# cuteboyqq/DPVO

Hardware: AMD Instinct MI355X
Metric: update-iterations/sec (altcorr+fastba) on 96-patch/2048-edge graph, 1→8 GPU (higher is better)
Workload: dtype f32; 1 GPU; cfg2: 96 patches/frame x 2048 edges, p=3, 4-level pyramid [1, 2, 4, 8], fp32 features, BA 2 iters; patches_per_frame=96, edges=2048, frames=12, radius=3, channels=128, feature_ring=36, parallelism=replicas x1

## Files before the change

### dpvo_amd/csrc/ba.hip

```cpp
#include "common.hpp"
#include "ba_device.hpp"

namespace dpvo {

constexpr int kSetupThreads = 1024;
constexpr int kIterThreads = 512;
constexpr int kIterWaves = kIterThreads / 64;
constexpr int kMaxSetupE = 16384;
constexpr int kMaxFree = 20;
constexpr int kPerThread = kMaxSetupE / kSetupThreads;
constexpr int kCtlBytes = 512;
constexpr int kSetupLds = 160 * 1024;
constexpr int kMarks = 2432;
constexpr int kLaunchMarks = 1664;
constexpr int kNoPose = 31;
constexpr int kEC = 16;

struct BaWs {
  int4* srec;
  int32_t* poff;
  int32_t* pu;
  uint32_t* pmask;
  int32_t* meta;
  int64_t* kx;
// ... 256 lines not shown
    work = pij + E;
#pragma unroll
    for (int k = 0; k < kPerThread; k++) {
      const int i = tid + k * T;
      if (i < E) {
        const int e = pe[k];
        const int64_t gi = A.ii[e], gj = A.jj[e];
        const int64_t pi = gi - t0, pj = gj - t0;
        const int ci = (pi >= 0 && pi < N) ? (int)pi : kNoPose;
        const int cj = (pj >= 0 && pj < N) ? (int)pj : kNoPose;
        pij[i] = ci | (cj << 8);
        work[i] = hd[k];
        w.srec[i] = make_int4(e, (int)gi, (int)gj, kv[k]);
      }
    }
    __syncthreads();
    nuniq = block_exclusive_scan(work, E, scr);
#pragma unroll
    for (int k = 0; k < kPerThread; k++) {
      const int i = tid + k * T;
      if (i < E) w.pu[i] = work[i] + hd[k] - 1;
      if (i < E && hd[k]) {
        w.kx[work[i]] = kv[k];
        w.poff[work[i]] = i;
      }
    }
    if (tid == 0) w.poff[nuniq] = E;
  }
  if (tid == 0) {
    w.meta[0] = nuniq;
    w.meta[1] = ctl[0] ? 2 : 0;
    w.meta[3] = A.num_patches;
    w.meta[4] = 0;
  }
  __syncthreads();
  trace(w.tmark, 41);
  for (int u = tid; u < nuniq; u += T) {
    unsigned mask = 0;
    for (int t = w.poff[u]; t < w.poff[u + 1]; t++) {
      const int c = pij[t];
      if ((c & 0xff) != kNoPose) mask |= 1u << (c & 0xff);
      if ((c >> 8) != kNoPose) mask |= 1u << (c >> 8);
    }
    w.pmask[u] = mask;
  }
  trace(w.tmark, 42);
}

#pragma clang fp contract(off)
__device__ __forceinline__ void edge_linearize(const float* poses, const float* patches, int P,
                                               float fx, float fy, float cx, float cy, float tx,
                                               float ty, float wx, float wy, int ix, int jx,
                                               int64_t kx, bool use_depth, float depth, float* o) {
  const float* pk = patches + (size_t)kx * 3 * P * P;
  const int c11 = P + 1;
  const float nx = (pk[c11] - cx) / fx;
  const float ny = (pk[P * P + c11] - cy) / fy;
  const float dz = use_depth ? depth : pk[2 * P * P + c11];
  bad::Lin L;
  bad::lin_edge(poses + 7 * (size_t)ix, poses + 7 * (size_t)jx, nx, ny, dz, tx, ty, wx, wy, fx, fy,
                cx, cy, L);
  o[0] = L.w[0];
  o[1] = L.w[1];
  o[2] = L.r[0];
  o[3] = L.r[1];
  o[4] = L.Jz[0];
  o[5] = L.Jz[1];
#pragma unroll
  for (int a = 0; a < 6; a++) {
    o[6 + a] = L.Ji[0][a];
    o[12 + a] = L.Ji[1][a];
    o[18 + a] = L.Jj[0][a];
    o[24 + a] = L.Jj[1][a];
  }
}

__global__ void reproject_kernel(const float* __restrict__ poses, const float* __restrict__ patches,
                                 const float* __restrict__ intrinsics,
                                 const int64_t* __restrict__ ii, const int64_t* __restrict__ jj,
                                 const int64_t* __restrict__ kk, int E, int P, int num_poses,
                                 int num_patches, float* __restrict__ coords,
                                 int* __restrict__ order, int N2) {
  if (order && blockIdx.x == gridDim.x - 1) {
    __shared__ int bins[kOrderBins + 1];
    const OrderIn q{poses, patches, intrinsics, ii, kk, P, num_poses, num_patches};
    edge_order_block(q, jj, E, N2, order, bins);
    return;
  }
  const int PP = P * P;
  const int t = blockIdx.x * blockDim.x + threadIdx.x;
  if (t >= E * PP) return;
  reproject_pixel(poses, patches, intrinsics, ii, jj, kk, t / PP, t % PP, P, num_poses,
                  num_patches, coords);
}
#pragma clang fp contract(fast)

__device__ __forceinline__ float retract_depth(const BaWs& w, const double* EC, const double* dX,
                                               int t0, int N, double lam, int u, float base) {
  double C = 0.0, Uu = 0.0, ex = 0.0;
  const int p1 = w.poff[u + 1];
#pragma unroll 2
  for (int t = w.poff[u]; t < p1; t++) {
    const double* ec = EC + kEC * (size_t)t;
    const int pi = (int)ec[14], pj = (int)ec[15];
    C += ec[12];
    Uu += ec[13];
    if (pi >= 0 && pi < N)
#pragma unroll
      for (int k = 0; k < 6; k++) ex += ec[k] * dX[6 * pi + k];
    if (pj >= 0 && pj < N)
#pragma unroll
      for (int k = 0; k < 6; k++) ex += ec[6 + k] * dX[6 * pj + k];
  }
  const float dz = (float)((1.0 / (C + lam)) * (Uu - ex));
  float d = base + dz;
  d = (d > 20.0f) ? 1.0f : d;
  return (float)fmax((double)d, 1e-4);
}

__global__ void __launch_bounds__(256) ba_lin_kernel(BaArgs A, BaWs w, int it) {
  const int t = blockIdx.x * blockDim.x + threadIdx.x;
  if (t == 0) w.lam[0] = A.lmbda[0];
  if (t >= A.E) return;
  const float fx = A.intrinsics[0], fy = A.intrinsics[1], cx = A.intrinsics[2],
              cy = A.intrinsics[3];
  const int4 r = w.srec[t];
  const int kmax = w.meta[3] - 1;
  float depth = 0.0f;
  if (it > 0) {
    const int u = w.pu[t], P = A.P;
    const float base = (it == 1)
                           ? A.patches[(size_t)min(r.w, kmax) * 3 * P * P + 2 * P * P]
                           : w.dbuf[(it - 1) & 1][u];
    depth = retract_depth(w, w.EC[(it - 1) & 1], w.dX, A.t0, A.N, (double)A.lmbda[0], u, base);
    if (t == w.poff[u]) w.dbuf[it & 1][u] = depth;
  }
  const float2 tg = reinterpret_cast<const float2*>(A.target)[r.x];
  const float2 wt = reinterpret_cast<const float2*>(A.weight)[r.x];
  const int ix = min(max(r.y, 0), A.num_poses - 1);
  const int jx = min(max(r.z, 0), A.num_poses - 1);
  float o[30];
  edge_linearize(A.poses, A.patches, A.P, fx, fy, cx, cy, tg.x, tg.y, wt.x, wt.y, ix, jx,
                 (int64_t)min(r.w, kmax), it > 0, depth, o);
  float4* Jo = reinterpret_cast<float4*>(w.J + 32 * (size_t)t);
#pragma unroll
  for (int k = 0; k < 7; k++) Jo[k] = make_float4(o[4 * k], o[4 * k + 1], o[4 * k + 2], o[4 * k + 3]);
  reinterpret_cast<float2*>(Jo + 7)[0] = make_float2(o[28], o[29]);
  double ec[kEC];
#pragma unroll
  for (int k = 0; k < 14; k++) ec[k] = 0.0;
#pragma unroll
  for (int row = 0; row < 2; row++) {
    const double wr = o[row];
    const float rr = o[2 + row], Jz = o[4 + row];
    const double wz = wr * Jz;
#pragma unroll
    for (int k = 0; k < 6; k++) {
      ec[k] -= wz * o[6 + 6 * row + k];
      ec[6 + k] += wz * o[18 + 6 * row + k];
    }
    ec[12] += wz * Jz;
    ec[13] += wr * rr * Jz;
  }
  ec[14] = (double)(r.y - A.t0);
  ec[15] = (double)(r.z - A.t0);
  double2* Eo = reinterpret_cast<double2*>(w.EC[it & 1] + kEC * (size_t)t);
#pragma unroll
// ... 947 lines not shown
```

### dpvo_amd/csrc/ba_window.hip

```cpp
#include <unistd.h>

#include <algorithm>
#include <chrono>
#include <cstdio>
#include <random>
#include <cstdlib>
#include <map>
#include <mutex>

#include "ba_solve.hpp"
#include "pyr_insert.hpp"

namespace dpvo {
namespace {
using namespace bad;

constexpr int kWT = 256;
constexpr int kPT = 512;
constexpr int kWMaxN = 16;
constexpr int kWMaxE = 10240;
constexpr int kWMaxG = 256;
constexpr int kWLds = 160 * 1024;
constexpr int kHistMax = 12288;
constexpr int kWSlots = 64;
// ... 325 lines not shown
              k64[lo] = b;
              k64[hi] = a;
            }
          } else {
            const unsigned a = k32[lo], b = k32[hi];
            if ((a > b) == up) {
              k32[lo] = b;
              k32[hi] = a;
            }
          }
        }
        __syncthreads();
      }
    for (int p = tid; p < E; p += T) {
      if (wide) {
        spos[p] = (unsigned short)(k64[p] & 0xffffffffull);
        head[p] = (p == 0 || (k64[p] >> 32) != (k64[p - 1] >> 32)) ? 1 : 0;
      } else {
        spos[p] = (unsigned short)(k32[p] & 0x3fffu);
        head[p] = (p == 0 || (k32[p] >> 14) != (k32[p - 1] >> 14)) ? 1 : 0;
      }
    }
  }
  __syncthreads();
  int* hd = (int*)U;
  for (int p = tid; p < E; p += T) hd[p] = head[p];
  __syncthreads();
  const int nuniq = fscan(hd, E, scr);
  for (int p = tid; p < E; p += T) {
    const int u1 = (p + 1 < E) ? hd[p + 1] : nuniq;
    const bool is_head = u1 != hd[p];
    const int u = u1 - 1;
    const int e = pos_edge[p];
    plan.epos[p] = e;
    if (is_head) {
      plan.poff[u] = p;
      plan.pkk[u] = (int)min(max(kk[e], (int64_t)0), (int64_t)kmaxc);
    }
  }
  if (tid == 0) plan.poff[nuniq] = E;
  unsigned* mask = (unsigned*)(U + sizeof(int) * cap);
  for (int u = tid; u < nuniq; u += T) mask[u] = 0u;
  __syncthreads();
  for (int p = tid; p < E; p += T) {
    const int u = ((p + 1 < E) ? hd[p + 1] : nuniq) - 1;
    const unsigned c = code[pos_edge[p]];
    const unsigned ci = c & 0xff, cj = c >> 8;
    const unsigned m = (ci != kFix ? 1u << ci : 0u) | (cj != kFix ? 1u << cj : 0u);
    if (m) atomicOr(&mask[u], m);
  }
  __syncthreads();
  for (int u = tid; u < nuniq; u += T) plan.pmask[u] = mask[u];
  if (tid == 0) {
    plan.meta[0] = nuniq;
    plan.meta[1] = ctl[2];
    plan.meta[2] = ctl[3];
    plan.meta[3] = 0;
    if (ctl[3] && plan.sink) atomicOr(plan.sink, ctl[3]);
    *plan.status = 0;
  }
}

__host__ __device__ constexpr int plan_shards(int E) {
  return E <= 512 ? 1 : ((E + 511) / 512 < kPlanShardMax ? (E + 511) / 512 : kPlanShardMax);
}
template <int kPer>
__device__ __forceinline__ void plan_sharded_k(const int64_t* __restrict__ ii,
                                             const int64_t* __restrict__ jj,
                                               const int64_t* __restrict__ kk, int E, int num_patches,
                                               int num_poses, int t0, int N, const Plan& plan,
                                               char* lds, int cap, size_t lds_bytes, int s, int S) {
  if (S <= 1) {
    if (s == 0) plan_block(ii, jj, kk, E, num_patches, num_poses, t0, N, plan, lds, cap);
    return;
  }
  if (plan.t0d) t0 = *plan.t0d;
  auto stamp = [&](int q) {
    if (s == 0 && threadIdx.x == 0) {
      reinterpret_cast<int64_t*>(plan.meta + 16)[q] = (int64_t)wall_clock64();
      if (q == 0 || q == 6) reinterpret_cast<int64_t*>(plan.meta + 16)[7 + (q == 6)] = (int64_t)clock64();
    }
  };
  stamp(0);
  const int tid = threadIdx.x, lane = tid & 63, T = kPT;
  int* ctl = (int*)lds;
  int* scr = ctl + 16;
  unsigned short* code = (unsigned short*)(lds + 256);
  unsigned short* spos = code + cap;
  int* hf = reinterpret_cast<int*>(spos + cap);
  int kv[kPer];
  plan_edges_pass<kPer>(ii, jj, kk, E, num_patches, num_poses, t0, N, ctl, code, kv);
  stamp(1);
  const int kmin = ctl[0], R = ctl[1] - kmin + 1;
  const int nlmax = (R + S - 1) / S;
  const bool fits = E > 0 && R <= kHistMax && E < (1 << 14) &&
                    256 + 4 * (size_t)cap + 4 * (size_t)R + 4 * (size_t)nlmax + 4 * kWMaxNB <= lds_bytes;
  if (!fits) {
    if (s == 0) {
      __syncthreads();
      plan_block(ii, jj, kk, E, num_patches, num_poses, t0, N, plan, lds, cap);
    }
    return;
  }
  const int lo = (int)((long long)R * s / S), hi = (int)((long long)R * (s + 1) / S), nl = hi - lo;
  unsigned* pm = reinterpret_cast<unsigned*>(hf + R);
  int* wl = reinterpret_cast<int*>(pm + nl);
  for (int v = tid; v < R; v += T) hf[v] = 0;
  for (int v = tid; v < nl; v += T) pm[v] = 0u;
  for (int v = tid; v < kWMaxNB; v += T) wl[v] = 0;
  if (tid == 0) {
    ctl[4] = 0;
    ctl[5] = 0;
    ctl[6] = 0;
  }
  __syncthreads();
  int nb = 0;
#pragma unroll
  for (int r = 0; r < kPer; r++) {
    const int e = tid + r * T;
    if (e >= E) continue;
    const int v = kv[r] - kmin;
    atomicAdd(&hf[v], 1);
    nb += v < lo ? 1 : 0;
  }
  __syncthreads();
  stamp(2);
  int ub = 0, nu = 0;
  for (int v = tid; v < R; v += T) {
    const int present = hf[v] > 0 ? 1 : 0;
    nu += present;
    ub += v < lo ? present : 0;
  }
  nb = wave_sum_i(nb);
  ub = wave_sum_i(ub);
  nu = wave_sum_i(nu);
  if (lane == 0) {
    atomicAdd(&ctl[4], nb);
    atomicAdd(&ctl[5], ub);
    atomicAdd(&ctl[6], nu);
  }
  int* hist = hf + lo;
  fscan(hist, nl, scr, 14);
  stamp(3);
  const int below = ctl[4], ubelow = ctl[5], nuniq = ctl[6];
#pragma unroll
  for (int r = 0; r < kPer; r++) {
    const int e = tid + r * T;
    const int v = kv[r] - kmin - lo;
    if (e >= E || v < 0 || v >= nl) continue;
    const int old = atomicAdd(&hist[v], 1 << 14);
    spos[old >> 14] = (unsigned short)e;
    const unsigned c = code[e], ci = c & 0xff, cj = c >> 8;
    const unsigned m = (ci != kFix ? 1u << ci : 0u) | (cj != kFix ? 1u << cj : 0u);
    if (m) atomicOr(&pm[old & 0x3fff], m);
  }
  __syncthreads();
  stamp(4);
  plan_block_work(nl, [&](int v, int& c, unsigned& m) {
    const int hv = hist[v];
    c = (hv >> 14) - (v == 0 ? 0 : (hist[v - 1] >> 14));
    m = pm[hv & 0x3fff];
  }, wl);
  stamp(5);
#pragma unroll
  for (int r = 0; r < kPer; r++) {
    const int e = tid + r * T;
    const int v = kv[r] - kmin - lo;
    if (e >= E || v < 0 || v >= nl) continue;
    const int hv = hist[v];
    const int b = hv >> 14, a = (v == 0) ? 0 : (hist[v - 1] >> 14);
    const int rank = bucket_rank(spos, a, b, e);
    plan.epos[below + a + rank] = e;
    if (rank == 0) {
      const int u = ubelow + (hv & 0x3fff);
      plan.poff[u] = below + a;
      plan.pkk[u] = kv[r];
      plan.pmask[u] = pm[hv & 0x3fff];
    }
  }
  __syncthreads();
  plan_store_work(plan, wl, s, N);
  if (tid == 0 && s == S - 1) plan.poff[nuniq] = E;
  if (tid == 0 && s == 0) {
    plan.meta[0] = nuniq;
    plan.meta[1] = ctl[2];
    plan.meta[2] = ctl[3];
    plan.meta[3] = S;
    if (ctl[3] && plan.sink) atomicOr(plan.sink, ctl[3]);
    *plan.status = 0;
  }
  stamp(6);
}

__device__ __forceinline__ void plan_sharded(const int64_t* __restrict__ ii,
                                             const int64_t* __restrict__ jj,
                                             const int64_t* __restrict__ kk, int E, int num_patches,
                                             int num_poses, int t0, int N, const Plan& plan,
                                             char* lds, int cap, size_t lds_bytes, int s, int S) {
  if (E <= 4 * kPT)
    plan_sharded_k<4>(ii, jj, kk, E, num_patches, num_poses, t0, N, plan, lds, cap, lds_bytes, s, S);
  else
    plan_sharded_k<kPlanPer>(ii, jj, kk, E, num_patches, num_poses, t0, N, plan, lds, cap,
                             lds_bytes, s, S);
}

__global__ void __launch_bounds__(kPT) ba_plan_kernel(const int64_t* __restrict__ ii,
                                                      const int64_t* __restrict__ jj,
                                                      const int64_t* __restrict__ kk, int E,
                                                      int num_patches, int num_poses, int t0, int N,
                                                      Plan plan) {
  extern __shared__ __attribute__((aligned(16))) char lds[];
  plan_sharded(ii, jj, kk, E, num_patches, num_poses, t0, N, plan, lds, kWMaxE, kWLds, blockIdx.x,
               gridDim.x);
}

struct RArgs {
  const float* poses;
  const float* patches;
  const float* intrinsics;
  const int64_t* ii;
  const int64_t* jj;
  const int64_t* kk;
  int E, P, num_poses, num_patches, N2, t0, N;
  float* coords;
  int* order;
  int nps;
  int64_t* marks;
};

__global__ void __launch_bounds__(kPT) reproject_plan_kernel(RArgs R, Plan plan) {
  extern __shared__ __attribute__((aligned(16))) char lds[];
  if ((int)blockIdx.x < R.nps) {
    plan_sharded(R.ii, R.jj, R.kk, R.E, R.num_patches, R.num_poses, R.t0, R.N, plan, lds, kWMaxE,
                 kWLds, blockIdx.x, R.nps);
    return;
  }
  if ((int)blockIdx.x == R.nps) {
    const OrderIn q{R.poses, R.patches, R.intrinsics, R.ii, R.kk, R.P, R.num_poses, R.num_patches};
    edge_order_block(q, R.jj, R.E, R.N2, R.order, reinterpret_cast<int*>(lds));
    return;
  }
  const int PP = R.P * R.P;
  const int t = (blockIdx.x - R.nps - 1) * kPT + threadIdx.x;
  if (t >= R.E * PP) return;
  reproject_pixel(R.poses, R.patches, R.intrinsics, R.ii, R.jj, R.kk, t / PP, t % PP, R.P,
                  R.num_poses, R.num_patches, R.coords);
}

struct InsArgs {
  const void* src;
  InsLevels lv;
  int L, C, H, W, gx, gy, ntile;
};

template <typename T>
__device__ __forceinline__ void reproject_plan_insert_body(const RArgs& R, const Plan& plan,
                                                           const InsArgs& I, int nrep, char* lds) {
  const int b = blockIdx.x, b0 = R.nps + 1;
  if (b <= R.nps) __builtin_amdgcn_s_setprio(3);
  if (b < R.nps) {
    plan_sharded(R.ii, R.jj, R.kk, R.E, R.num_patches, R.num_poses, R.t0, R.N, plan, lds,
                 plan_cap(R.E), plan_lds_bytes(plan_cap(R.E)), b, R.nps);
    return;
  }
  if (b == R.nps) {
    const OrderIn q{R.poses, R.patches, R.intrinsics, R.ii, R.kk, R.P, R.num_poses, R.num_patches};
    edge_order_block(q, R.jj, R.E, R.N2, R.order, reinterpret_cast<int*>(lds));
    return;
  }
  if (b < b0 + nrep) {
    const int PP = R.P * R.P;
    const int t = (b - b0) * kPT + threadIdx.x;
    if (t >= R.E * PP) return;
    reproject_pixel(R.poses, R.patches, R.intrinsics, R.ii, R.jj, R.kk, t / PP, t % PP, R.P,
                    R.num_poses, R.num_patches, R.coords);
    return;
  }
  static_assert(kPT == 512, "two 256-thread insertion tiles per workgroup");
  const int half = threadIdx.x >> 8, t = 2 * (b - b0 - nrep) + half;
  const bool act = t < I.ntile;
  const int tt = act ? t : 0;
  float* tile = reinterpret_cast<float*>(lds) + half * kInsTC * kInsCS;
  ins_tile<T>(static_cast<const T*>(I.src), I.lv, I.L, I.C, I.H, I.W, tt % I.gx,
              (tt / I.gx) % I.gy, tt / (I.gx * I.gy), threadIdx.x & 255, act, tile);
}

template <typename T>
__global__ void __launch_bounds__(kPT) reproject_plan_insert_kernel(RArgs R, Plan plan, InsArgs I,
                                                                    int nrep) {
  extern __shared__ __attribute__((aligned(16))) char lds[];
  const bool mk = R.marks && blockIdx.x < 256;
  if (mk && threadIdx.x == 0) R.marks[2 * blockIdx.x] = (int64_t)wall_clock64();
  reproject_plan_insert_body<T>(R, plan, I, nrep, lds);
  if (mk) {
    __syncthreads();
    if (threadIdx.x == 0) R.marks[2 * blockIdx.x + 1] = (int64_t)wall_clock64();
  }
}

struct WL {
  int* ctl;
  float* pose;
  double* dX;
  unsigned short* tri;
  int* roff;
  float2* nxy;
  float* dep;
  float* dbase;
  double2* qu;
  int* pkx;
  unsigned short* ec;
  unsigned short* rp;
  int* eid;
  float4* tw;
  float* ej;
  char* region;
  __device__ __forceinline__ void ld_ej(const float* ejg, int E, int q, int par, float4& e0,
                                        float4& e1, float4& e2) const {
    if (ej) {
      const float4* e4 = reinterpret_cast<const float4*>(ej + 12 * (size_t)q);
      e0 = e4[0];
      e1 = e4[1];
      e2 = e4[2];
    } else {
      const __amdgpu_buffer_rsrc_t rs = __builtin_amdgcn_make_buffer_rsrc(
          const_cast<float*>(ejg), 0, (int)(sizeof(float) * 24 * (size_t)E), kBufDword3);
      const int o = (int)(sizeof(float) * 12 * ((size_t)par * E + eid[q]));
      e0 = __builtin_bit_cast(float4, __builtin_amdgcn_raw_buffer_load_b128(rs, o, 0, kSc1));
      e1 = __builtin_bit_cast(float4, __builtin_amdgcn_raw_buffer_load_b128(rs, o + 16, 0, kSc1));
      e2 = __builtin_bit_cast(float4, __builtin_amdgcn_raw_buffer_load_b128(rs, o + 32, 0, kSc1));
    }
  }
};

enum { cNrel = 0, cNrp = 1, cFmin = 2, cFail = 3, cTimeout = 4, cCap = 5, cFailAny = 6, cLMulti = 7,
       cScan = 16 };

__device__ __forceinline__ double edges_etdx(const WL& L, const WArgs& A, int q0, int q1, int par,
                                             int N) {
  constexpr int kEb = 4;
  double ex = 0.0;
  for (int qb = q0; qb < q1; qb += kEb) {
    float4 e[kEb][3];
    unsigned cc[kEb];
#pragma unroll
    for (int u = 0; u < kEb; u++) {
      const int q = min(qb + u, q1 - 1);
      cc[u] = L.ec[q];
      L.ld_ej(A.ejg, A.E, q, par, e[u][0], e[u][1], e[u][2]);
    }
#pragma unroll
    for (int u = 0; u < kEb; u++) {
      const bool live = qb + u < q1;
      const unsigned si = cc[u] & 0xff, sj = cc[u] >> 8;
      const unsigned nm = (unsigned)max(N - 1, 0);
      const double* dj = L.dX + 6 * min(sj, nm);
      const double* di = L.dX + 6 * min(si, nm);
      const float4 e0 = e[u][0], e1 = e[u][1], e2 = e[u][2];
      const double tj = (double)e0.x * dj[0] + (double)e0.y * dj[1] + (double)e0.z * dj[2] +
                        (double)e0.w * dj[3] + (double)e1.x * dj[4] + (double)e1.y * dj[5];
      const double ti = (double)e1.z * di[0] + (double)e1.w * di[1] + (double)e2.x * di[2] +
                        (double)e2.y * di[3] + (double)e2.z * di[4] + (double)e2.w * di[5];
      ex += (live && sj < (unsigned)N) ? tj : 0.0;
      ex += (live && si < (unsigned)N) ? ti : 0.0;
    }
  }
  return ex;
}
__device__ __forceinline__ double patch_etdx(const WL& L, const WArgs& A, int ri, int par, int N) {
  return edges_etdx(L, A, L.roff[ri], L.roff[ri + 1], par, N);
}
// ... 1013 lines not shown
  g_sink[dev] = sink;
}

void ba_window_plan_offsets(int E, int64_t* out) {
  out[0] = 0;
  out[1] = out[0] + (int64_t)al256w(sizeof(int) * (size_t)E);
  out[2] = out[1] + (int64_t)al256w(sizeof(int) * (size_t)(E + 1));
  out[3] = out[2] + (int64_t)al256w(sizeof(unsigned) * (size_t)E);
  out[4] = out[3] + (int64_t)al256w(sizeof(int) * (size_t)E);
}

static Plan plan_view(char* scratch, int E, int* status) {
  Plan p;
  char* s = scratch;
  p.epos = (int*)s;
  s += al256w(sizeof(int) * (size_t)E);
  p.poff = (int*)s;
  s += al256w(sizeof(int) * (size_t)(E + 1));
  p.pmask = (unsigned*)s;
  s += al256w(sizeof(unsigned) * (size_t)E);
  p.pkk = (int*)s;
  s += al256w(sizeof(int) * (size_t)E);
  p.meta = (int*)s;
  p.status = status;
  p.sink = sink_for_device();
  p.t0d = nullptr;
  return p;
}

static void set_attrs() {
  static bool attr = false;
  if (!attr) {
    (void)hipFuncSetAttribute((const void*)ba_window_kernel,
                              hipFuncAttributeMaxDynamicSharedMemorySize, kWLds);
    (void)hipFuncSetAttribute((const void*)ba_plan_kernel,
                              hipFuncAttributeMaxDynamicSharedMemorySize, kWLds);
    (void)hipFuncSetAttribute((const void*)reproject_plan_kernel,
                              hipFuncAttributeMaxDynamicSharedMemorySize, kWLds);
    (void)hipFuncSetAttribute((const void*)reproject_plan_insert_kernel<float>,
                              hipFuncAttributeMaxDynamicSharedMemorySize, kWLds);
    (void)hipFuncSetAttribute((const void*)reproject_plan_insert_kernel<__half>,
                              hipFuncAttributeMaxDynamicSharedMemorySize, kWLds);
    attr = true;
  }
}

int ba_window_plan(const int64_t* ii, const int64_t* jj, const int64_t* kk, int E, int num_patches,
                   int num_poses, int t0, int t1, char* scratch, int* status, void* stream,
                   const int* t0d) {
  set_attrs();
  Plan plan = plan_view(scratch, E, status);
  plan.t0d = t0d;
  hipLaunchKernelGGL(ba_plan_kernel, dim3(plan_shards(E)), dim3(kPT), kWLds, as_stream(stream), ii, jj, kk, E,
                     num_patches, num_poses, t0, t1 - t0, plan);
  return launch_status();
}

int ba_window_reproject_plan(const float* poses, const float* patches, const float* intrinsics,
                             const int64_t* ii, const int64_t* jj, const int64_t* kk, int E, int P,
                             int num_poses, int num_patches, int N2, float* coords, int* order,
                             int t0, int t1, char* scratch, int* status, void* stream,
                             const int* t0d) {
  set_attrs();
  Plan plan = plan_view(scratch, E, status);
  plan.t0d = t0d;
  RArgs r;
  r.marks = nullptr;
  r.poses = poses;
  r.patches = patches;
  r.intrinsics = intrinsics;
  r.ii = ii;
  r.jj = jj;
  r.kk = kk;
  r.E = E;
  r.P = P;
  r.num_poses = num_poses;
  r.num_patches = num_patches;
  r.N2 = N2;
  r.t0 = t0;
  r.N = t1 - t0;
  r.coords = coords;
  r.order = order;
  r.nps = plan_shards(E);
  const int total = E * P * P;
  hipLaunchKernelGGL(reproject_plan_kernel, dim3(r.nps + 1 + (total + kPT - 1) / kPT), dim3(kPT), kWLds,
                     as_stream(stream), r, plan);
  return launch_status();
}

int ba_window_reproject_plan_insert(const float* poses, const float* patches,
                                    const float* intrinsics, const int64_t* ii, const int64_t* jj,
                                    const int64_t* kk, int E, int P, int num_poses,
                                    int num_patches, int N2, float* coords, int* order, int t0,
                                    int t1, char* scratch, int* status, const void* src,
                                    void* const* dst, const int* scale, int L, int C, int H, int W,
                                    int half, int64_t* marks, void* stream) {
  set_attrs();
  Plan plan = plan_view(scratch, E, status);
  plan.t0d = nullptr;
  RArgs r;
  r.marks = marks;
  r.poses = poses;
  r.patches = patches;
  r.intrinsics = intrinsics;
  r.ii = ii;
  r.jj = jj;
  r.kk = kk;
  r.E = E;
  r.P = P;
  r.num_poses = num_poses;
  r.num_patches = num_patches;
  r.N2 = N2;
  r.t0 = t0;
  r.N = t1 - t0;
  r.coords = coords;
  r.order = order;
  r.nps = plan_shards(E);
  InsArgs I = {};
  I.src = src;
  I.L = L;
  I.C = C;
  I.H = H;
  I.W = W;
  I.lv.mem = 1;
  for (int l = 0; l < L; l++) {
    I.lv.dst[l] = dst[l];
    I.lv.s[l] = scale[l];
  }
  I.gx = (W + kInsTX - 1) / kInsTX;
  I.gy = (H + kInsTY - 1) / kInsTY;
  I.ntile = I.gx * I.gy * ((C + kInsTC - 1) / kInsTC);
  const int nrep = (E * P * P + kPT - 1) / kPT;
  const dim3 grid(r.nps + 1 + nrep + (I.ntile + 1) / 2);
  size_t lds = plan_lds_bytes(plan_cap(E));
  lds = std::max(lds, sizeof(float) * 2 * kInsTC * kInsCS);
  lds = std::max(lds, sizeof(int) * (size_t)(kOrderBins + 2));
  if (half)
    hipLaunchKernelGGL(reproject_plan_insert_kernel<__half>, grid, dim3(kPT), lds,
                       as_stream(stream), r, plan, I, nrep);
  else
    hipLaunchKernelGGL(reproject_plan_insert_kernel<float>, grid, dim3(kPT), lds,
                       as_stream(stream), r, plan, I, nrep);
  return launch_status();
}

int ba_window_run(float* poses, float* patches, const float* intrinsics, const float* target,
                  const float* weight, const float* lmbda, const int64_t* ii, const int64_t* jj,
                  const int64_t* kk, int E, int P, int num_poses, int num_patches, int t0, int t1,
                  int iterations, char* scratch, int* status, int64_t* marks, double* dxo,
                  void* stream, const int* t0d = nullptr);

int ba_window_launch(float* poses, float* patches, const float* intrinsics, const float* target,
                     const float* weight, const float* lmbda, const int64_t* ii, const int64_t* jj,
                     const int64_t* kk, int E, int P, int num_poses, int num_patches, int t0, int t1,
                     int iterations, char* scratch, int* status, int64_t* marks, double* dxo,
                     void* stream) {
  const int rc = ba_window_plan(ii, jj, kk, E, num_patches, num_poses, t0, t1, scratch, status,
                                stream, nullptr);
  if (rc) return rc;
  return ba_window_run(poses, patches, intrinsics, target, weight, lmbda, ii, jj, kk, E, P,
                       num_poses, num_patches, t0, t1, iterations, scratch, status, marks, dxo,
                       stream);
}

int ba_window_run(float* poses, float* patches, const float* intrinsics, const float* target,
                  const float* weight, const float* lmbda, const int64_t* ii, const int64_t* jj,
                  const int64_t* kk, int E, int P, int num_poses, int num_patches, int t0, int t1,
                  int iterations, char* scratch, int* status, int64_t* marks, double* dxo,
                  void* stream, const int* t0d) {
  set_attrs();
  if (iterations > 63) return DPVO_ERR_UNSUPPORTED;
  const int N = t1 - t0;
  const WGrid w = window_grid(E, N);
  hipStream_t st = as_stream(stream);
  WArgs a;
  a.flags = wflag_slot(st);
  if (!a.flags) return DPVO_ERR_LAUNCH;
  a.plan = plan_view(scratch, E, status);
  char* s = scratch + al256w(sizeof(int) * (size_t)E) + al256w(sizeof(int) * (size_t)(E + 1)) +
            al256w(sizeof(unsigned) * (size_t)E) + al256w(sizeof(int) * (size_t)E) +
            al256w(kMetaBytes);
  a.part = (double*)s;
  s += al256w(sizeof(double) * 2 * kPartPad * (size_t)w.G);
  a.gran = (v4u*)s;
  s += al256w((size_t)16 * gran_count(w));
  a.ejg = (float*)s;
  a.poses = poses;
  a.patches = patches;
  a.intrinsics = intrinsics;
  a.target = target;
  a.weight = weight;
  a.lmbda = lmbda;
  a.ii = ii;
  a.jj = jj;
  a.kk = kk;
  a.E = E;
  a.P = P;
  a.num_poses = num_poses;
  a.num_patches = num_patches;
  a.t0 = t0;
  a.t0d = t0d;
  a.N = N;
  a.iters = iterations;
  a.NB = w.NB;
  a.Sd = w.Sd;
  a.So = w.So;
  a.G = w.G;
  a.status = status;
  a.sink = a.plan.sink;
  a.marks = marks;
  a.dxo = dxo;
  a.salt = granule_salt();
  hipLaunchKernelGGL(ba_window_kernel, dim3(w.G), dim3(kWT), kWLds, st, a);
  return launch_status();
}

}
```

### dpvo_amd/csrc/common.hpp

```cpp
#pragma once

#include <hip/hip_fp16.h>
#include <hip/hip_runtime.h>
#include <stdint.h>

#include "dpvo_hot.h"

#define DPVO_EXPORT extern "C" __attribute__((visibility("default")))

namespace dpvo {

constexpr int kWave = 64;
constexpr int kMaxDevices = 64;

inline hipStream_t as_stream(void* s) { return reinterpret_cast<hipStream_t>(s); }

inline int launch_status() {
  hipError_t e = hipGetLastError();
  return e == hipSuccess ? DPVO_OK : DPVO_ERR_LAUNCH;
}

template <typename T>
struct Acc { using type = float; };
template <>
struct Acc<double> { using type = double; };

__device__ __forceinline__ float to_acc(float v) { return v; }
__device__ __forceinline__ float to_acc(__half v) { return __half2float(v); }
__device__ __forceinline__ double to_acc(double v) { return v; }

template <typename T>
__device__ __forceinline__ T from_acc(float v);
template <>
__device__ __forceinline__ float from_acc<float>(float v) { return v; }
template <>
__device__ __forceinline__ __half from_acc<__half>(float v) { return __float2half(v); }
template <>
__device__ __forceinline__ double from_acc<double>(float v) { return (double)v; }
__device__ __forceinline__ double from_acc_d(double v) { return v; }

__device__ __forceinline__ int ifloor_safe(float v) {
  float f = floorf(v);
  f = fminf(fmaxf(f, -1.0e8f), 1.0e8f);
  return (int)f;
}

__device__ __forceinline__ int wave_uniform(int v) { return __builtin_amdgcn_readfirstlane(v); }

__device__ __forceinline__ void wave_lds_sync() {
  __builtin_amdgcn_fence(__ATOMIC_ACQ_REL, "wavefront", "local");
  __builtin_amdgcn_wave_barrier();
}

template <typename Op>
__device__ __forceinline__ int wave_scan_dpp(int x, int id, Op op) {
  x = op(x, __builtin_amdgcn_update_dpp(id, x, 0x111, 0xf, 0xf, false));
  x = op(x, __builtin_amdgcn_update_dpp(id, x, 0x112, 0xf, 0xf, false));
  x = op(x, __builtin_amdgcn_update_dpp(id, x, 0x114, 0xf, 0xf, false));
  x = op(x, __builtin_amdgcn_update_dpp(id, x, 0x118, 0xf, 0xf, false));
  x = op(x, __builtin_amdgcn_update_dpp(id, x, 0x142, 0xa, 0xf, false));
  x = op(x, __builtin_amdgcn_update_dpp(id, x, 0x143, 0xc, 0xf, false));
  return x;
}
__device__ __forceinline__ int wave_incl_sum(int x) {
  return wave_scan_dpp(x, 0, [](int a, int b) { return a + b; });
}
__device__ __forceinline__ int wave_sum_i(int x) {
  return __builtin_amdgcn_readlane(wave_incl_sum(x), 63);
}
__device__ __forceinline__ int wave_min_i(int x) {
  return __builtin_amdgcn_readlane(
      wave_scan_dpp(x, 0x7fffffff, [](int a, int b) { return a < b ? a : b; }), 63);
}
__device__ __forceinline__ int wave_max_i(int x) {
  return __builtin_amdgcn_readlane(
      wave_scan_dpp(x, (int)0x80000000, [](int a, int b) { return a > b ? a : b; }), 63);
}

template <typename T>
__device__ __forceinline__ T wave_sum(T v) {
#pragma unroll
  for (int o = 32; o > 0; o >>= 1) v += __shfl_xor(v, o, kWave);
  return v;
}

#pragma clang fp contract(off)
__device__ __forceinline__ void actSO3(const float* q, const float* X, float* Y) {
  float uv[3];
  uv[0] = 2.0f * (q[1] * X[2] - q[2] * X[1]);
  uv[1] = 2.0f * (q[2] * X[0] - q[0] * X[2]);
  uv[2] = 2.0f * (q[0] * X[1] - q[1] * X[0]);
  Y[0] = X[0] + q[3] * uv[0] + (q[1] * uv[2] - q[2] * uv[1]);
  Y[1] = X[1] + q[3] * uv[1] + (q[2] * uv[0] - q[0] * uv[2]);
  Y[2] = X[2] + q[3] * uv[2] + (q[0] * uv[1] - q[1] * uv[0]);
}

__device__ __forceinline__ void actSE3(const float* t, const float* q, const float* X, float* Y) {
  actSO3(q, X, Y);
  Y[3] = X[3];
  Y[0] += X[3] * t[0];
  Y[1] += X[3] * t[1];
  Y[2] += X[3] * t[2];
}

__device__ __forceinline__ void adjSE3(const float* t, const float* q, const float* X, float* Y) {
  float qinv[4] = {-q[0], -q[1], -q[2], q[3]};
  actSO3(qinv, &X[0], &Y[0]);
  actSO3(qinv, &X[3], &Y[3]);
  float u[3], v[3];
  u[0] = t[2] * X[1] - t[1] * X[2];
  u[1] = t[0] * X[2] - t[2] * X[0];
  u[2] = t[1] * X[0] - t[0] * X[1];
  actSO3(qinv, u, v);
  Y[3] += v[0];
  Y[4] += v[1];
  Y[5] += v[2];
}

__device__ __forceinline__ void relSE3(const float* ti, const float* qi, const float* tj,
                                       const float* qj, float* tij, float* qij) {
  qij[0] = -qj[3] * qi[0] + qj[0] * qi[3] - qj[1] * qi[2] + qj[2] * qi[1];
  qij[1] = -qj[3] * qi[1] + qj[1] * qi[3] - qj[2] * qi[0] + qj[0] * qi[2];
  qij[2] = -qj[3] * qi[2] + qj[2] * qi[3] - qj[0] * qi[1] + qj[1] * qi[0];
  qij[3] = qj[3] * qi[3] + qj[0] * qi[0] + qj[1] * qi[1] + qj[2] * qi[2];
  actSO3(qij, ti, tij);
  tij[0] = tj[0] - tij[0];
  tij[1] = tj[1] - tij[1];
  tij[2] = tj[2] - tij[2];
}

__device__ __forceinline__ void expSO3(const float* phi, float* q) {
  float theta_sq = phi[0] * phi[0] + phi[1] * phi[1] + phi[2] * phi[2];
  float theta_p4 = theta_sq * theta_sq;
  float theta = sqrtf(theta_sq);
// ... 44 lines not shown
}

__device__ __forceinline__ void retrSE3(const float* xi, const float* t, const float* q, float* t1,
                                        float* q1) {
  float dt[3] = {0, 0, 0};
  float dq[4] = {0, 0, 0, 1};
  expSE3(xi, dt, dq);
  q1[0] = dq[3] * q[0] + dq[0] * q[3] + dq[1] * q[2] - dq[2] * q[1];
  q1[1] = dq[3] * q[1] + dq[1] * q[3] + dq[2] * q[0] - dq[0] * q[2];
  q1[2] = dq[3] * q[2] + dq[2] * q[3] + dq[0] * q[1] - dq[1] * q[0];
  q1[3] = dq[3] * q[3] - dq[0] * q[0] - dq[1] * q[1] - dq[2] * q[2];
  actSO3(dq, t, t1);
  t1[0] += dt[0];
  t1[1] += dt[1];
  t1[2] += dt[2];
}

__device__ __forceinline__ void reproject_uv(const float* __restrict__ poses,
                                             const float* __restrict__ patches,
                                             const float* __restrict__ intrinsics,
                                             const int64_t* __restrict__ ii,
                                             const int64_t* __restrict__ jj,
                                             const int64_t* __restrict__ kk, int n, int pix, int P,
                                             int num_poses, int num_patches, float& u, float& v) {
  const int PP = P * P;
  const float fx = intrinsics[0], fy = intrinsics[1], cx = intrinsics[2], cy = intrinsics[3];
  const int ix = (int)min(max(ii[n], (int64_t)0), (int64_t)num_poses - 1);
  const int jx = (int)min(max(jj[n], (int64_t)0), (int64_t)num_poses - 1);
  const int64_t kx = min(max(kk[n], (int64_t)0), (int64_t)num_patches - 1);
  const float* pi = poses + 7 * (size_t)ix;
  const float* pj = poses + 7 * (size_t)jx;
  float ti[3] = {pi[0], pi[1], pi[2]}, qi[4] = {pi[3], pi[4], pi[5], pi[6]};
  float tj[3] = {pj[0], pj[1], pj[2]}, qj[4] = {pj[3], pj[4], pj[5], pj[6]};
  float tij[3], qij[4];
  relSE3(ti, qi, tj, qj, tij, qij);
  const float* pk = patches + (size_t)kx * 3 * PP;
  float Xi[4], Xj[4];
  Xi[0] = (pk[pix] - cx) / fx;
  Xi[1] = (pk[PP + pix] - cy) / fy;
  Xi[2] = 1.0f;
  Xi[3] = pk[2 * PP + pix];
  actSE3(tij, qij, Xi, Xj);
  u = fx * (Xj[0] / Xj[2]) + cx;
  v = fy * (Xj[1] / Xj[2]) + cy;
}

__device__ __forceinline__ void reproject_pixel(const float* __restrict__ poses,
                                                const float* __restrict__ patches,
                                                const float* __restrict__ intrinsics,
                                                const int64_t* __restrict__ ii,
                                                const int64_t* __restrict__ jj,
                                                const int64_t* __restrict__ kk, int n, int pix,
                                                int P, int num_poses, int num_patches,
                                                float* __restrict__ coords) {
  const int PP = P * P;
  float u, v;
  reproject_uv(poses, patches, intrinsics, ii, jj, kk, n, pix, P, num_poses, num_patches, u, v);
  coords[((size_t)n * 2 + 0) * PP + pix] = u;
  coords[((size_t)n * 2 + 1) * PP + pix] = v;
}

#pragma clang fp contract(fast)

struct OrderIn {
  const float* poses;
  const float* patches;
  const float* intrinsics;
  const int64_t* ii;
  const int64_t* kk;
  int P, num_poses, num_patches;
};
constexpr int kOrderBins = 1024;
constexpr int kOrderBands = 16;
__device__ __forceinline__ int edge_order_key(const OrderIn& q, const int64_t* __restrict__ jj,
                                              int e, int nf) {
  const int64_t f = jj[e];
  float u, v;
  const int c = (q.P / 2) * q.P + q.P / 2;
  reproject_uv(q.poses, q.patches, q.intrinsics, q.ii, jj, q.kk, e, c, q.P, q.num_poses,
               q.num_patches, u, v);
  const int band = v >= 0.0f ? (int)fminf(v * (1.0f / 16.0f), (float)(kOrderBands - 1)) : 0;
  return ((f >= 0 && f < nf) ? (int)f : nf - 1) * kOrderBands + band;
}
__device__ inline void edge_order_block(const OrderIn& q, const int64_t* __restrict__ jj, int E,
                                        int N2, int* __restrict__ order, int* bins) {
  const int tid = threadIdx.x, T = blockDim.x;
  const int nf = min(max(N2, 1), kOrderBins / kOrderBands), nb = nf * kOrderBands;
  if (E <= 0) return;
  auto keys4 = [&](int e0, int (&k)[4]) __attribute__((always_inline)) {
#pragma unroll
    for (int r = 0; r < 4; r++) k[r] = edge_order_key(q, jj, min(e0 + r * T, E - 1), nf);
  };
  int k0[4];
  keys4(tid, k0);
  for (int b = tid; b <= nb; b += T) bins[b] = 0;
  __syncthreads();
  for (int e0 = tid; e0 < E; e0 += 4 * T) {
    int k[4];
    if (e0 == tid) {
#pragma unroll
      for (int r = 0; r < 4; r++) k[r] = k0[r];
    } else {
      keys4(e0, k);
    }
#pragma unroll
    for (int r = 0; r < 4; r++)
      if (e0 + r * T < E) atomicAdd(&bins[k[r]], 1);
  }
  __syncthreads();
  if (tid < 64) {
    int carry = 0;
    for (int b0 = 0; b0 < nb; b0 += 64) {
      const int b = b0 + tid;
      const int c = (b < nb) ? bins[b] : 0;
      int x = c;
#pragma unroll
      for (int o = 1; o < 64; o <<= 1) {
        const int y = __shfl_up(x, o, 64);
        if (tid >= o) x += y;
      }
      if (b < nb) bins[b] = carry + x - c;
      carry += __shfl(x, 63, 64);
    }
  }
  __syncthreads();
  for (int e0 = tid; e0 < E; e0 += 4 * T) {
    int k[4];
    if (e0 == tid) {
#pragma unroll
      for (int r = 0; r < 4; r++) k[r] = k0[r];
    } else {
      keys4(e0, k);
    }
#pragma unroll
    for (int r = 0; r < 4; r++)
      if (e0 + r * T < E) order[atomicAdd(&bins[k[r]], 1)] = e0 + r * T;
  }
}

}
```

Baseline: 8768 update-iterations/s.

## Restructure plan sharding, edge ordering scan, and block placement in reproject-plan kernels

The sharded planner now does a single fused load pass over ii/jj/kk with a hashed full-range histogram, replacing the separate edge pass, per-shard histogram and fscan with a block-wide packed count/unique prefix scan, and iterates output by sorted position. Edge ordering replaces the single-wave serial scan with a block-wide scan and reuses keys computed once. Plan/order blocks are spread across block indices so they land on different compute units, launch bounds request two workgroups per CU, and raw barriers replace __syncthreads. These target the latency of the serial planning chain that gates each update iteration, at the cost of more complex index mapping, a hash mask that falls back when the key range exceeds the table, and added register pressure.

```diff
diff --git a/dpvo_amd/csrc/ba.hip b/dpvo_amd/csrc/ba.hip
--- a/dpvo_amd/csrc/ba.hip
+++ b/dpvo_amd/csrc/ba.hip
@@ -362,7 +362,7 @@
                                  int num_patches, float* __restrict__ coords,
                                  int* __restrict__ order, int N2) {
   if (order && blockIdx.x == gridDim.x - 1) {
-    __shared__ int bins[kOrderBins + 1];
+    __shared__ int bins[kOrderLds];
     const OrderIn q{poses, patches, intrinsics, ii, kk, P, num_poses, num_patches};
     edge_order_block(q, jj, E, N2, order, bins);
     return;
diff --git a/dpvo_amd/csrc/ba_window.hip b/dpvo_amd/csrc/ba_window.hip
--- a/dpvo_amd/csrc/ba_window.hip
+++ b/dpvo_amd/csrc/ba_window.hip
@@ -431,20 +431,87 @@
     }
   };
   stamp(0);
-  const int tid = threadIdx.x, lane = tid & 63, T = kPT;
+  const int tid = threadIdx.x, lane = tid & 63, wid = tid >> 6, T = kPT;
   int* ctl = (int*)lds;
   int* scr = ctl + 16;
-  unsigned short* code = (unsigned short*)(lds + 256);
-  unsigned short* spos = code + cap;
-  int* hf = reinterpret_cast<int*>(spos + cap);
+  unsigned short* spos = (unsigned short*)(lds + 256);
+  unsigned short* sv = spos + cap;
+  int* wl = reinterpret_cast<int*>(sv + cap);
+  int* hf = wl + kWMaxNB;
+  const int avail = (int)((lds_bytes - 256 - 4 * (size_t)cap) / 4) - kWMaxNB;
+  int Z = 16384;
+  while (Z > 64 && Z + ((Z / S + 8) & ~3) > avail) Z >>= 1;
+  const int zm = Z - 1, pmN = (Z / S + 8) & ~3;
+  unsigned* pm = reinterpret_cast<unsigned*>(hf + Z);
+  const int kmaxc = num_patches - 1;
+  constexpr int kRound = kPer % 5 == 0 ? 5 : kPer;
+  static_assert(kPer % kRound == 0, "load rounds");
   int kv[kPer];
-  plan_edges_pass<kPer>(ii, jj, kk, E, num_patches, num_poses, t0, N, ctl, code, kv);
-  stamp(1);
-  const int kmin = ctl[0], R = ctl[1] - kmin + 1;
-  const int nlmax = (R + S - 1) / S;
-  const bool fits = E > 0 && R <= kHistMax && E < (1 << 14) &&
-                    256 + 4 * (size_t)cap + 4 * (size_t)R + 4 * (size_t)nlmax + 4 * kWMaxNB <= lds_bytes;
-  if (!fits) {
+  unsigned mk[kPer];
+  int kmin = 0x7fffffff, kmax = -1, fmin = 0x7fffffff, bad = 0;
+#pragma unroll
+  for (int r = 0; r < kPer; r++) {
+    kv[r] = 0;
+    mk[r] = 0u;
+  }
+#pragma unroll
+  for (int r0 = 0; r0 < kPer; r0 += kRound) {
+    if (r0 > 0 && r0 * T >= E) break;
+    int64_t vk[kRound], vi[kRound], vj[kRound];
+#pragma unroll
+    for (int r = 0; r < kRound; r++) {
+      const int e = min(tid + (r0 + r) * T, E - 1);
+      vk[r] = kk[e];
+      vi[r] = ii[e];
+      vj[r] = jj[e];
+    }
+    if (r0 == 0) {
+      int4* z = reinterpret_cast<int4*>(wl);
+      for (int q = tid; q < (kWMaxNB + Z + pmN) / 4; q += T) z[q] = make_int4(0, 0, 0, 0);
+      if (tid == 0) {
+        ctl[0] = 0x7fffffff;
+        ctl[1] = -1;
+        ctl[2] = 0x7fffffff;
+        ctl[3] = 0;
+      }
+      lds_barrier();
+      stamp(1);
+    }
+#pragma unroll
+    for (int r = 0; r < kRound; r++) {
+      const int e = tid + (r0 + r) * T;
+      if (e >= E) continue;
+      int64_t v = vk[r];
+      if (v < 0 || v > kmaxc) {
+        bad = 1;
+        v = v < 0 ? 0 : kmaxc;
+      }
+      kmin = min(kmin, (int)v);
+      kmax = max(kmax, (int)v);
+      kv[r0 + r] = (int)v;
+      atomicAdd(&hf[(int)v & zm], 1);
+      const int64_t gi = vi[r], gj = vj[r];
+      const bool fi = gi >= t0 && gi < t0 + N, fj = gj >= t0 && gj < t0 + N;
+      if (!fi) fmin = min(fmin, (int)min(max(gi, (int64_t)0), (int64_t)num_poses - 1));
+      if (!fj) fmin = min(fmin, (int)min(max(gj, (int64_t)0), (int64_t)num_poses - 1));
+      mk[r0 + r] = (fi ? 1u << (int)(gi - t0) : 0u) | (fj ? 1u << (int)(gj - t0) : 0u);
+    }
+  }
+  kmin = wave_min_i(kmin);
+  kmax = wave_max_i(kmax);
+  fmin = wave_min_i(fmin);
+  bad = wave_max_i(bad);
+  if (lane == 0) {
+    atomicMin(&ctl[0], kmin);
+    atomicMax(&ctl[1], kmax);
+    atomicMin(&ctl[2], fmin);
+    if (bad) atomicOr(&ctl[3], kStClamp);
+  }
+  lds_barrier();
+  stamp(2);
+  kmin = ctl[0];
+  const int R = ctl[1] - kmin + 1;
+  if (__builtin_expect(R > Z || E >= (1 << 14), 0)) {
     if (s == 0) {
       __syncthreads();
       plan_block(ii, jj, kk, E, num_patches, num_poses, t0, N, plan, lds, cap);
@@ -452,82 +519,74 @@
     return;
   }
   const int lo = (int)((long long)R * s / S), hi = (int)((long long)R * (s + 1) / S), nl = hi - lo;
-  unsigned* pm = reinterpret_cast<unsigned*>(hf + R);
-  int* wl = reinterpret_cast<int*>(pm + nl);
-  for (int v = tid; v < R; v += T) hf[v] = 0;
-  for (int v = tid; v < nl; v += T) pm[v] = 0u;
-  for (int v = tid; v < kWMaxNB; v += T) wl[v] = 0;
-  if (tid == 0) {
-    ctl[4] = 0;
-    ctl[5] = 0;
-    ctl[6] = 0;
-  }
-  __syncthreads();
-  int nb = 0;
-#pragma unroll
-  for (int r = 0; r < kPer; r++) {
-    const int e = tid + r * T;
-    if (e >= E) continue;
-    const int v = kv[r] - kmin;
-    atomicAdd(&hf[v], 1);
-    nb += v < lo ? 1 : 0;
-  }
-  __syncthreads();
-  stamp(2);
-  int ub = 0, nu = 0;
-  for (int v = tid; v < R; v += T) {
-    const int present = hf[v] > 0 ? 1 : 0;
-    nu += present;
-    ub += v < lo ? present : 0;
-  }
-  nb = wave_sum_i(nb);
-  ub = wave_sum_i(ub);
-  nu = wave_sum_i(nu);
-  if (lane == 0) {
-    atomicAdd(&ctl[4], nb);
-    atomicAdd(&ctl[5], ub);
-    atomicAdd(&ctl[6], nu);
-  }
-  int* hist = hf + lo;
-  fscan(hist, nl, scr, 14);
+  const int per = (R + T - 1) / T, v0 = tid * per, v1 = min(v0 + per, R);
+  int sum = 0;
+  for (int k0 = v0; k0 < v1; k0 += 4) {
+    int c[4];
+#pragma unroll
+    for (int j = 0; j < 4; j++) c[j] = hf[(kmin + min(k0 + j, v1 - 1)) & zm];
+#pragma unroll
+    for (int j = 0; j < 4; j++) sum += k0 + j < v1 ? (c[j] << 14) | (c[j] > 0 ? 1 : 0) : 0;
+  }
+  const int incl = wave_incl_sum(sum);
+  if (lane == 63) scr[wid] = incl;
+  lds_barrier();
+  int total = 0, run = incl - sum;
+#pragma unroll
+  for (int w = 0; w < kPT / 64; w++) {
+    const int x = scr[w];
+    total += x;
+    run += w < wid ? x : 0;
+  }
+  for (int k0 = v0; k0 < v1; k0 += 4) {
+    int c[4];
+#pragma unroll
+    for (int j = 0; j < 4; j++) c[j] = hf[(kmin + min(k0 + j, v1 - 1)) & zm];
+#pragma unroll
+    for (int j = 0; j < 4; j++) {
+      const int v = k0 + j;
+      if (v >= v1) continue;
+      if (v >= lo && v < hi) hf[(kmin + v) & zm] = run;
+      if (v == lo) ctl[4] = run >> 14;
+      if (v == hi) ctl[5] = run >> 14;
+      run += (c[j] << 14) | (c[j] > 0 ? 1 : 0);
+    }
+  }
+  lds_barrier();
   stamp(3);
-  const int below = ctl[4], ubelow = ctl[5], nuniq = ctl[6];
+  const int nuniq = total & 0x3fff;
+  const int below = ctl[4], top = hi < R ? ctl[5] : total >> 14;
 #pragma unroll
   for (int r = 0; r < kPer; r++) {
     const int e = tid + r * T;
     const int v = kv[r] - kmin - lo;
     if (e >= E || v < 0 || v >= nl) continue;
-    const int old = atomicAdd(&hist[v], 1 << 14);
-    spos[old >> 14] = (unsigned short)e;
-    const unsigned c = code[e], ci = c & 0xff, cj = c >> 8;
-    const unsigned m = (ci != kFix ? 1u << ci : 0u) | (cj != kFix ? 1u << cj : 0u);
-    if (m) atomicOr(&pm[old & 0x3fff], m);
-  }
-  __syncthreads();
+    const int p = atomicAdd(&hf[kv[r] & zm], 1 << 14) >> 14;
+    spos[p] = (unsigned short)e;
+    sv[p] = (unsigned short)v;
+    if (mk[r]) atomicOr(&pm[v], mk[r]);
+  }
+  lds_barrier();
   stamp(4);
   plan_block_work(nl, [&](int v, int& c, unsigned& m) {
-    const int hv = hist[v];
-    c = (hv >> 14) - (v == 0 ? 0 : (hist[v - 1] >> 14));
-    m = pm[hv & 0x3fff];
+    c = (hf[(kmin + lo + v) & zm] >> 14) - (v == 0 ? below : (hf[(kmin + lo + v - 1) & zm] >> 14));
+    m = pm[v];
   }, wl);
   stamp(5);
-#pragma unroll
-  for (int r = 0; r < kPer; r++) {
-    const int e = tid + r * T;
-    const int v = kv[r] - kmin - lo;
-    if (e >= E || v < 0 || v >= nl) continue;
-    const int hv = hist[v];
-    const int b = hv >> 14, a = (v == 0) ? 0 : (hist[v - 1] >> 14);
+  for (int p = below + tid; p < top; p += T) {
+    const int e = spos[p], v = sv[p];
+    const int hv = hf[(kmin + lo + v) & zm];
+    const int b = hv >> 14, a = v == 0 ? below : (hf[(kmin + lo + v - 1) & zm] >> 14);
     const int rank = bucket_rank(spos, a, b, e);
-    plan.epos[below + a + rank] = e;
+    plan.epos[a + rank] = e;
     if (rank == 0) {
-      const int u = ubelow + (hv & 0x3fff);
-      plan.poff[u] = below + a;
-      plan.pkk[u] = kv[r];
-      plan.pmask[u] = pm[hv & 0x3fff];
-    }
-  }
-  __syncthreads();
+      const int u = hv & 0x3fff;
+      plan.poff[u] = a;
+      plan.pkk[u] = kmin + lo + v;
+      plan.pmask[u] = pm[v];
+    }
+  }
+  lds_barrier();
   plan_store_work(plan, wl, s, N);
   if (tid == 0 && s == S - 1) plan.poff[nuniq] = E;
   if (tid == 0 && s == 0) {
@@ -541,16 +600,23 @@
   stamp(6);
 }
 
+__device__ __forceinline__ void plan_sharded_long(const int64_t* __restrict__ ii,
+                                               const int64_t* __restrict__ jj,
+                                               const int64_t* __restrict__ kk, int E, int num_patches,
+                                               int num_poses, int t0, int N, const Plan& plan,
+                                               char* lds, int cap, size_t lds_bytes, int s, int S) {
+  plan_sharded_k<kPlanPer>(ii, jj, kk, E, num_patches, num_poses, t0, N, plan, lds, cap, lds_bytes,
+                           s, S);
+}
 __device__ __forceinline__ void plan_sharded(const int64_t* __restrict__ ii,
                                              const int64_t* __restrict__ jj,
                                              const int64_t* __restrict__ kk, int E, int num_patches,
                                              int num_poses, int t0, int N, const Plan& plan,
                                              char* lds, int cap, size_t lds_bytes, int s, int S) {
-  if (E <= 4 * kPT)
+  if (__builtin_expect(E <= 4 * kPT, 1))
     plan_sharded_k<4>(ii, jj, kk, E, num_patches, num_poses, t0, N, plan, lds, cap, lds_bytes, s, S);
   else
-    plan_sharded_k<kPlanPer>(ii, jj, kk, E, num_patches, num_poses, t0, N, plan, lds, cap,
-                             lds_bytes, s, S);
+    plan_sharded_long(ii, jj, kk, E, num_patches, num_poses, t0, N, plan, lds, cap, lds_bytes, s, S);
 }
 
 __global__ void __launch_bounds__(kPT) ba_plan_kernel(const int64_t* __restrict__ ii,
@@ -574,23 +640,36 @@
   float* coords;
   int* order;
   int nps;
+  int spread;
   int64_t* marks;
 };
 
+__device__ __forceinline__ int launch_chain(const RArgs& R, int b) {
+  if (!R.spread) return b <= R.nps ? b : -1;
+  const int c = 2 * (b >> 3) + (b & 7);
+  return ((b & 7) < 2 && c <= R.nps) ? c : -1;
+}
+__device__ __forceinline__ int launch_rest(const RArgs& R, int b) {
+  if (!R.spread) return b - R.nps - 1;
+  return b - min(R.nps + 1, 2 * (b >> 3) + min(b & 7, 2));
+}
+inline int launch_spread(int nps, int grid) { return grid >= 8 * (nps / 2) + 2 ? 1 : 0; }
+
 __global__ void __launch_bounds__(kPT) reproject_plan_kernel(RArgs R, Plan plan) {
   extern __shared__ __attribute__((aligned(16))) char lds[];
-  if ((int)blockIdx.x < R.nps) {
+  const int chain = launch_chain(R, blockIdx.x);
+  if (chain >= 0 && chain < R.nps) {
     plan_sharded(R.ii, R.jj, R.kk, R.E, R.num_patches, R.num_poses, R.t0, R.N, plan, lds, kWMaxE,
-                 kWLds, blockIdx.x, R.nps);
+                 kWLds, chain, R.nps);
     return;
   }
-  if ((int)blockIdx.x == R.nps) {
+  if (chain == R.nps) {
     const OrderIn q{R.poses, R.patches, R.intrinsics, R.ii, R.kk, R.P, R.num_poses, R.num_patches};
     edge_order_block(q, R.jj, R.E, R.N2, R.order, reinterpret_cast<int*>(lds));
     return;
   }
   const int PP = R.P * R.P;
-  const int t = (blockIdx.x - R.nps - 1) * kPT + threadIdx.x;
+  const int t = launch_rest(R, blockIdx.x) * kPT + threadIdx.x;
   if (t >= R.E * PP) return;
   reproject_pixel(R.poses, R.patches, R.intrinsics, R.ii, R.jj, R.kk, t / PP, t % PP, R.P,
                   R.num_poses, R.num_patches, R.coords);
@@ -605,28 +684,29 @@
 template <typename T>
 __device__ __forceinline__ void reproject_plan_insert_body(const RArgs& R, const Plan& plan,
                                                            const InsArgs& I, int nrep, char* lds) {
-  const int b = blockIdx.x, b0 = R.nps + 1;
-  if (b <= R.nps) __builtin_amdgcn_s_setprio(3);
-  if (b < R.nps) {
+  const int chain = launch_chain(R, blockIdx.x);
+  if (chain >= 0) __builtin_amdgcn_s_setprio(3);
+  if (chain >= 0 && chain < R.nps) {
     plan_sharded(R.ii, R.jj, R.kk, R.E, R.num_patches, R.num_poses, R.t0, R.N, plan, lds,
-                 plan_cap(R.E), plan_lds_bytes(plan_cap(R.E)), b, R.nps);
+                 plan_cap(R.E), plan_lds_bytes(plan_cap(R.E)), chain, R.nps);
     return;
   }
-  if (b == R.nps) {
+  if (chain == R.nps) {
     const OrderIn q{R.poses, R.patches, R.intrinsics, R.ii, R.kk, R.P, R.num_poses, R.num_patches};
     edge_order_block(q, R.jj, R.E, R.N2, R.order, reinterpret_cast<int*>(lds));
     return;
   }
-  if (b < b0 + nrep) {
+  const int b = launch_rest(R, blockIdx.x);
+  if (b < nrep) {
     const int PP = R.P * R.P;
-    const int t = (b - b0) * kPT + threadIdx.x;
+    const int t = b * kPT + threadIdx.x;
     if (t >= R.E * PP) return;
     reproject_pixel(R.poses, R.patches, R.intrinsics, R.ii, R.jj, R.kk, t / PP, t % PP, R.P,
                     R.num_poses, R.num_patches, R.coords);
     return;
   }
   static_assert(kPT == 512, "two 256-thread insertion tiles per workgroup");
-  const int half = threadIdx.x >> 8, t = 2 * (b - b0 - nrep) + half;
+  const int half = threadIdx.x >> 8, t = 2 * (b - nrep) + half;
   const bool act = t < I.ntile;
   const int tt = act ? t : 0;
   float* tile = reinterpret_cast<float*>(lds) + half * kInsTC * kInsCS;
@@ -635,7 +715,7 @@
 }
 
 template <typename T>
-__global__ void __launch_bounds__(kPT) reproject_plan_insert_kernel(RArgs R, Plan plan, InsArgs I,
+__global__ void __launch_bounds__(kPT, 2) reproject_plan_insert_kernel(RArgs R, Plan plan, InsArgs I,
                                                                     int nrep) {
   extern __shared__ __attribute__((aligned(16))) char lds[];
   const bool mk = R.marks && blockIdx.x < 256;
@@ -1815,9 +1895,10 @@
   r.coords = coords;
   r.order = order;
   r.nps = plan_shards(E);
-  const int total = E * P * P;
-  hipLaunchKernelGGL(reproject_plan_kernel, dim3(r.nps + 1 + (total + kPT - 1) / kPT), dim3(kPT), kWLds,
-                     as_stream(stream), r, plan);
+  const int total = E * P * P, grid = r.nps + 1 + (total + kPT - 1) / kPT;
+  r.spread = launch_spread(r.nps, grid);
+  hipLaunchKernelGGL(reproject_plan_kernel, dim3(grid), dim3(kPT), kWLds, as_stream(stream), r,
+                     plan);
   return launch_status();
 }
 
@@ -1865,9 +1946,10 @@
   I.ntile = I.gx * I.gy * ((C + kInsTC - 1) / kInsTC);
   const int nrep = (E * P * P + kPT - 1) / kPT;
   const dim3 grid(r.nps + 1 + nrep + (I.ntile + 1) / 2);
+  r.spread = launch_spread(r.nps, (int)grid.x);
   size_t lds = plan_lds_bytes(plan_cap(E));
   lds = std::max(lds, sizeof(float) * 2 * kInsTC * kInsCS);
-  lds = std::max(lds, sizeof(int) * (size_t)(kOrderBins + 2));
+  lds = std::max(lds, sizeof(int) * (size_t)kOrderLds);
   if (half)
     hipLaunchKernelGGL(reproject_plan_insert_kernel<__half>, grid, dim3(kPT), lds,
                        as_stream(stream), r, plan, I, nrep);
diff --git a/dpvo_amd/csrc/common.hpp b/dpvo_amd/csrc/common.hpp
--- a/dpvo_amd/csrc/common.hpp
+++ b/dpvo_amd/csrc/common.hpp
@@ -50,6 +50,12 @@
 __device__ __forceinline__ void wave_lds_sync() {
   __builtin_amdgcn_fence(__ATOMIC_ACQ_REL, "wavefront", "local");
   __builtin_amdgcn_wave_barrier();
+}
+
+__device__ __forceinline__ void lds_barrier() {
+  __builtin_amdgcn_fence(__ATOMIC_RELEASE, "workgroup", "local");
+  __builtin_amdgcn_s_barrier();
+  __builtin_amdgcn_fence(__ATOMIC_ACQUIRE, "workgroup", "local");
 }
 
 template <typename Op>
@@ -260,60 +266,56 @@
   const int band = v >= 0.0f ? (int)fminf(v * (1.0f / 16.0f), (float)(kOrderBands - 1)) : 0;
   return ((f >= 0 && f < nf) ? (int)f : nf - 1) * kOrderBands + band;
 }
+__device__ __forceinline__ void edge_order_rest(const OrderIn& q, const int64_t* __restrict__ jj, int E,
+                                             int nf, int* __restrict__ order, int* bins) {
+  const int tid = threadIdx.x, T = blockDim.x;
+  for (int e0 = tid + 4 * T; e0 < E; e0 += 4 * T) {
+    int k[4];
+#pragma unroll
+    for (int r = 0; r < 4; r++) k[r] = edge_order_key(q, jj, min(e0 + r * T, E - 1), nf);
+#pragma unroll
+    for (int r = 0; r < 4; r++) {
+      if (e0 + r * T >= E) continue;
+      const int p = atomicAdd(&bins[k[r]], 1);
+      if (order) order[p] = e0 + r * T;
+    }
+  }
+}
+constexpr int kOrderLds = kOrderBins + 1 + 16;
 __device__ inline void edge_order_block(const OrderIn& q, const int64_t* __restrict__ jj, int E,
                                         int N2, int* __restrict__ order, int* bins) {
-  const int tid = threadIdx.x, T = blockDim.x;
+  const int tid = threadIdx.x, T = blockDim.x, lane = tid & 63, wid = tid >> 6;
   const int nf = min(max(N2, 1), kOrderBins / kOrderBands), nb = nf * kOrderBands;
+  int* scr = bins + kOrderBins + 1;
   if (E <= 0) return;
-  auto keys4 = [&](int e0, int (&k)[4]) __attribute__((always_inline)) {
-#pragma unroll
-    for (int r = 0; r < 4; r++) k[r] = edge_order_key(q, jj, min(e0 + r * T, E - 1), nf);
-  };
   int k0[4];
-  keys4(tid, k0);
+#pragma unroll
+  for (int r = 0; r < 4; r++) k0[r] = edge_order_key(q, jj, min(tid + r * T, E - 1), nf);
   for (int b = tid; b <= nb; b += T) bins[b] = 0;
-  __syncthreads();
-  for (int e0 = tid; e0 < E; e0 += 4 * T) {
-    int k[4];
-    if (e0 == tid) {
-#pragma unroll
-      for (int r = 0; r < 4; r++) k[r] = k0[r];
-    } else {
-      keys4(e0, k);
-    }
-#pragma unroll
-    for (int r = 0; r < 4; r++)
-      if (e0 + r * T < E) atomicAdd(&bins[k[r]], 1);
+  lds_barrier();
+#pragma unroll
+  for (int r = 0; r < 4; r++)
+    if (tid + r * T < E) atomicAdd(&bins[k0[r]], 1);
+  if (__builtin_expect(E > 4 * T, 0)) edge_order_rest(q, jj, E, nf, nullptr, bins);
+  lds_barrier();
+  const int per = (nb + T - 1) / T, b0 = min(tid * per, nb), b1 = min(b0 + per, nb);
+  int sum = 0;
+  for (int b = b0; b < b1; b++) sum += bins[b];
+  const int incl = wave_incl_sum(sum);
+  if (lane == 63) scr[wid] = incl;
+  lds_barrier();
+  int run = incl - sum;
+  for (int w = 0; w < wid; w++) run += scr[w];
+  for (int b = b0; b < b1; b++) {
+    const int c = bins[b];
+    bins[b] = run;
+    run += c;
   }
-  __syncthreads();
-  if (tid < 64) {
-    int carry = 0;
-    for (int b0 = 0; b0 < nb; b0 += 64) {
-      const int b = b0 + tid;
-      const int c = (b < nb) ? bins[b] : 0;
-      int x = c;
-#pragma unroll
-      for (int o = 1; o < 64; o <<= 1) {
-        const int y = __shfl_up(x, o, 64);
-        if (tid >= o) x += y;
-      }
-      if (b < nb) bins[b] = carry + x - c;
-      carry += __shfl(x, 63, 64);
-    }
-  }
-  __syncthreads();
-  for (int e0 = tid; e0 < E; e0 += 4 * T) {
-    int k[4];
-    if (e0 == tid) {
-#pragma unroll
-      for (int r = 0; r < 4; r++) k[r] = k0[r];
-    } else {
-      keys4(e0, k);
-    }
-#pragma unroll
-    for (int r = 0; r < 4; r++)
-      if (e0 + r * T < E) order[atomicAdd(&bins[k[r]], 1)] = e0 + r * T;
-  }
-}
-
-}
+  lds_barrier();
+#pragma unroll
+  for (int r = 0; r < 4; r++)
+    if (tid + r * T < E) order[atomicAdd(&bins[k0[r]], 1)] = tid + r * T;
+  if (__builtin_expect(E > 4 * T, 0)) edge_order_rest(q, jj, E, nf, order, bins);
+}
+
+}
```

Measured after the change: 8906 update-iterations/s (median of 6 runs). 1.02x the previous value.
